# brockpat/JKMP22-Machine-Learning-and-the-Implementable-Efficient-Frontier-Replication

Measured on AMD Instinct MI355X. Metric: PFML hp×window solves/sec (whole node); full grid-search wall-clock, S&P500, higher is better.
Workload: dtype fp64; 1 GPU; global_batch=42824, seq_len=710, parallelism=dp1, dist_backend=none, device=AMD Radeon Graphics, outputs_finite=True, includes_s4_inputs=False, ridge_solve_dtype=fp64 (lambda = 0 / rank-deficient systems: bf16 cannot carry them, SURVEY 7.4), hip_graph=True

## Files before the change

### jkmp22-machine-learning-and-the-implementable-efficient-frontier-replication_amd/csrc/segsum.hip

```cpp
#include "common.h"

namespace {

__device__ __forceinline__ double* seg_slot(double* out, double* scratch, int g, int s, int nseg,
                                            int skip, int64_t PP) {
  return s < skip ? scratch + ((int64_t)g * skip + s) * PP
                  : out + ((int64_t)g * (nseg - skip) + (s - skip)) * PP;
}

__global__ __launch_bounds__(256) void wsum_upper_kernel(const double* __restrict__ X, int P,
                                                         int T, const int* __restrict__ seg_start,
                                                         const int* __restrict__ seg_stop,
                                                         int nseg, int skip,
                                                         double* __restrict__ out,
                                                         double* __restrict__ scratch) {
  const int i = blockIdx.x, s = blockIdx.y, g = blockIdx.z;
  const int a = seg_start[s], b = seg_stop[s];
  const int64_t PP = (int64_t)P * P;
  const double* src = X + (int64_t)g * T * PP + (int64_t)i * P;
  double* dst = seg_slot(out, scratch, g, s, nseg, skip, PP) + (int64_t)i * P;
  for (int j = i + threadIdx.x; j < P; j += 256) {
    double acc[4] = {0.0, 0.0, 0.0, 0.0};
    int tm = a;
    for (; tm + 4 <= b; tm += 4) {
#pragma unroll
      for (int u = 0; u < 4; ++u) acc[u] += src[(int64_t)(tm + u) * PP + j];
    }
    for (; tm < b; ++tm) acc[0] += src[(int64_t)tm * PP + j];
    dst[j] = (acc[0] + acc[1]) + (acc[2] + acc[3]);
  }
}

constexpr int WV_COLS = 64, WV_SEG = 128, WV_T = 1024, WV_RG = WV_T / WV_COLS;
template <int COLS, int RG>
__device__ __forceinline__ void wvec_segsums(const double* src, int64_t E, const int* seg_start,
                                             const int* seg_stop, int nseg, int ry, int lc,
                                             double (*part)[COLS]) {
  for (int s = ry; s < nseg; s += RG) {
    const int a = seg_start[s], b = seg_stop[s];
    double acc[8] = {0.0, 0.0, 0.0, 0.0, 0.0, 0.0, 0.0, 0.0};
    for (int tm = a; tm < b; tm += 8) {
      double x[8];
#pragma unroll
      for (int u = 0; u < 8; ++u) x[u] = (tm + u < b) ? src[(int64_t)(tm + u) * E] : 0.0;
#pragma unroll
      for (int u = 0; u < 8; ++u) acc[u] += x[u];
    }
    part[s][lc] = ((acc[0] + acc[1]) + (acc[2] + acc[3])) + ((acc[4] + acc[5]) + (acc[6] + acc[7]));
  }
}

}

namespace {

__device__ __forceinline__ bool tile_upper(int I, int J, int i, int j, int r, int c, int P) {
  return i < P && j < P && (I != J || c >= r);
}

__global__ __launch_bounds__(256) void wsum_chunk_totals_kernel(
    int P, int nseg, int skip, const double* __restrict__ out, const double* __restrict__ scratch,
    int nlc, const int* __restrict__ cs, const int* __restrict__ ce, const int* __restrict__ slot,
    double* __restrict__ tot, int64_t tstride) {
  const int g = blockIdx.y, lc = blockIdx.z;
  int tile = blockIdx.x;
  const int nt = (P + 31) / 32;
  int I = 0;
  while (tile >= nt - I) { tile -= nt - I; ++I; }
  const int J = I + tile;
  const int64_t PP = (int64_t)P * P;
  const int t = threadIdx.x, c = t & 31, r0 = t >> 5;
  double acc[4] = {0.0, 0.0, 0.0, 0.0};
  const int s0 = cs[lc], s1 = ce[lc];
  double nx[4];
  auto fetch = [&](int s) {
    const double* o = seg_slot(const_cast<double*>(out), const_cast<double*>(scratch), g, s,
                               nseg, skip, PP);
#pragma unroll
    for (int q = 0; q < 4; ++q) {
      const int i = min(I * 32 + r0 + 8 * q, P - 1), j = min(J * 32 + c, P - 1);
      nx[q] = o[(int64_t)i * P + j];
    }
  };
  if (s0 < s1) fetch(s0);
  for (int s = s0; s < s1; ++s) {
    double cur[4];
#pragma unroll
    for (int q = 0; q < 4; ++q) cur[q] = nx[q];
    if (s + 1 < s1) fetch(s + 1);
#pragma unroll
    for (int q = 0; q < 4; ++q) {
      const int r = r0 + 8 * q, i = I * 32 + r, j = J * 32 + c;
      if (tile_upper(I, J, i, j, r, c, P)) acc[q] += cur[q];
    }
  }
  double* d = tot + (int64_t)slot[lc] * tstride + (int64_t)g * PP;
#pragma unroll
  for (int q = 0; q < 4; ++q) {
    const int r = r0 + 8 * q, i = I * 32 + r, j = J * 32 + c;
    if (tile_upper(I, J, i, j, r, c, P)) d[(int64_t)i * P + j] = acc[q];
  }
}

__global__ __launch_bounds__(256) void wsum_chunk_prefix_kernel(
    int P, int nseg, int skip, double* __restrict__ out, double* __restrict__ scratch, int C,
    const int* __restrict__ sb, const int* __restrict__ sy, const int* __restrict__ ys,
    const int* __restrict__ ye, const double* __restrict__ tot, int64_t tstride, int clast) {
  __shared__ double Ts[32][33];
  const int g = blockIdx.y, ch = blockIdx.z;
  const int s0 = ys[ch], s1 = ye[ch];
  if (s0 >= s1) return;
  int tile = blockIdx.x;
  const int nt = (P + 31) / 32;
  int I = 0;
  while (tile >= nt - I) { tile -= nt - I; ++I; }
  const int J = I + tile;
  const int64_t PP = (int64_t)P * P;
  const int t = threadIdx.x, c = t & 31, r0 = t >> 5;
  const double* tg = tot + (int64_t)g * PP;
  double nx[4];
  auto fetch = [&](int s) {
    const double* o = seg_slot(out, scratch, g, s, nseg, skip, PP);
#pragma unroll
    for (int q = 0; q < 4; ++q) {
      const int i = min(I * 32 + r0 + 8 * q, P - 1), j = min(J * 32 + c, P - 1);
      nx[q] = o[(int64_t)i * P + j];
    }
  };
  fetch(s0);
  double acc[4] = {0.0, 0.0, 0.0, 0.0};
  const int nk = C + ch;
  for (int k0 = 0; k0 < nk; k0 += 8) {
    double v[8][4];
#pragma unroll
    for (int u = 0; u < 8; ++u) {
      const int k = min(k0 + u, nk - 1);
      const double* o = tg + (int64_t)(k < C ? sb[k] : sy[k - C]) * tstride;
#pragma unroll
      for (int q = 0; q < 4; ++q) {
        const int i = min(I * 32 + r0 + 8 * q, P - 1), j = min(J * 32 + c, P - 1);
        v[u][q] = o[(int64_t)i * P + j];
      }
    }
#pragma unroll
    for (int u = 0; u < 8; ++u) {
      if (k0 + u < nk) {
#pragma unroll
        for (int q = 0; q < 4; ++q) {
          const int r = r0 + 8 * q, i = I * 32 + r, j = J * 32 + c;
          if (tile_upper(I, J, i, j, r, c, P)) acc[q] += v[u][q];
        }
      }
    }
  }
  for (int s = s0; s < s1; ++s) {
    double cur[4];
#pragma unroll
    for (int q = 0; q < 4; ++q) cur[q] = nx[q];
    if (s + 1 < s1) fetch(s + 1);
#pragma unroll
    for (int q = 0; q < 4; ++q) {
      const int r = r0 + 8 * q, i = I * 32 + r, j = J * 32 + c;
      const double v = tile_upper(I, J, i, j, r, c, P) ? cur[q] : 0.0;
      acc[q] += v;
      Ts[r][c] = acc[q];
    }
    __syncthreads();
    if (s >= skip) {
      double* w = seg_slot(out, scratch, g, s, nseg, skip, PP);
#pragma unroll
      for (int q = 0; q < 4; ++q) {
        const int r = r0 + 8 * q;
        const int i = I * 32 + r, j = J * 32 + c;
        if (i < P && j < P) w[(int64_t)i * P + j] = (I != J || c >= r) ? Ts[r][c] : Ts[c][r];
        const int i2 = J * 32 + r, j2 = I * 32 + c;
        if (I != J && i2 < P && j2 < P) w[(int64_t)i2 * P + j2] = Ts[c][r];
      }
    }
    __syncthreads();
  }
}

__global__ __launch_bounds__(WV_T) void wvec_chunk_kernel(
    const double* __restrict__ X, int64_t E, int T, const int* __restrict__ seg_start,
    const int* __restrict__ seg_stop, int nseg, int skip, int mode, int nlc,
    const int* __restrict__ cs, const int* __restrict__ ce, const int* __restrict__ slot, int C,
    const int* __restrict__ sb, const int* __restrict__ sy, const int* __restrict__ ys,
    const int* __restrict__ ye, int clast, double* __restrict__ tot, int64_t tstride,
    double* __restrict__ out) {
  __shared__ double part[WV_SEG][WV_COLS];
  const int lc = threadIdx.x % WV_COLS, ry = threadIdx.x / WV_COLS;
  const int g = blockIdx.y, col = blockIdx.x * WV_COLS + lc;
  const bool cv = col < E;
  const double* src = X + (int64_t)g * T * E + (cv ? col : 0);
  wvec_segsums<WV_COLS, WV_RG>(src, E, seg_start, seg_stop, nseg, ry, lc, part);
  __syncthreads();
  if (ry != 0 || !cv) return;
  double* tg = tot + (int64_t)g * E + col;
  if (mode == 0) {
    for (int k = 0; k < nlc; ++k) {
      double acc = 0.0;
      for (int s = cs[k]; s < ce[k]; ++s) acc += part[s][lc];
      tg[(int64_t)slot[k] * tstride] = acc;
    }
    return;
  }
  double pc = 0.0;
  for (int k = 0; k < C; ++k) pc += tg[(int64_t)sb[k] * tstride];
  double* o = out + (int64_t)g * (nseg - skip) * E + col;
  for (int ch = 0; ch <= clast; ++ch) {
    double acc = pc;
    for (int s = ys[ch]; s < ye[ch]; ++s) {
      acc += part[s][lc];
      if (s >= skip) o[(int64_t)(s - skip) * E] = acc;
    }
    if (ch < clast) pc += tg[(int64_t)sy[ch] * tstride];
  }
}

}

extern "C" hipError_t pfml_wsum_chunk_totals(const double* X, int P, int T, int G,
                                             const int* seg_start, const int* seg_stop, int nseg,
                                             int skip, double* out, double* scratch, int nlc,
                                             const int* idx, double* tot, int64_t tstride,
                                             hipStream_t st) {
  if (nseg <= 0 || P <= 0 || G <= 0) return hipSuccess;
  if (skip < 0 || skip > nseg || (skip > 0 && scratch == nullptr)) return hipErrorInvalidValue;
  hipLaunchKernelGGL(wsum_upper_kernel, dim3(P, nseg, G), dim3(256), 0, st, X, P, T, seg_start,
                     seg_stop, nseg, skip, out, scratch);
  if (nlc > 0) {
    const int nt = (P + 31) / 32;
    hipLaunchKernelGGL(wsum_chunk_totals_kernel, dim3(nt * (nt + 1) / 2, G, nlc), dim3(256), 0, st, P,
                       nseg, skip, out, scratch, nlc, idx, idx + nlc, idx + 2 * nlc, tot,
                       tstride);
  }
  return hipGetLastError();
}

extern "C" hipError_t pfml_wsum_chunk_prefix(int P, int G, int nseg, int skip, double* out,
                                             double* scratch, int C, const int* cidx,
                                             const double* tot, int64_t tstride, int clast,
                                             hipStream_t st) {
  if (nseg <= 0 || P <= 0 || G <= 0 || clast < 0) return hipSuccess;
  const int nt = (P + 31) / 32;
  hipLaunchKernelGGL(wsum_chunk_prefix_kernel, dim3(nt * (nt + 1) / 2, G, clast + 1), dim3(256), 0, st, P,
                     nseg, skip, out, scratch, C, cidx, cidx + C, cidx + 2 * C, cidx + 3 * C, tot,
                     tstride, clast);
  return hipGetLastError();
}

namespace {
constexpr int OP_T = 256, OP_R = 8, OP_C = 64, OP_LD = OP_C + 2;
constexpr int OP_VC = 32, OP_VRG = OP_T / OP_VC;
static_assert(OP_T == OP_R * OP_C / 2, "one thread per column pair of the tile");
static_assert(2 * OP_R * OP_LD <= WV_SEG * OP_VC, "the tile buffers fit the vector job's LDS");

typedef double op_d2 __attribute__((ext_vector_type(2)));
struct __attribute__((aligned(8))) op_pair { double x, y; };

template <bool FULL>
__device__ __forceinline__ op_d2 op_load(const double* p, bool v0, bool v1) {
  op_d2 r = {0.0, 0.0};
  if (FULL) {
    const op_pair q = *reinterpret_cast<const op_pair*>(p);
    r.x = q.x;
    r.y = q.y;
  } else {
    if (v0) r.x = p[0];
    if (v1) r.y = p[1];
  }
  return r;
}

template <bool FULL>
__device__ __forceinline__ void op_store(double* p, bool v0, bool v1, double x, double y) {
  if (FULL) {
    op_pair q = {x, y};
    *reinterpret_cast<op_pair*>(p) = q;
  } else {
    if (v0) p[0] = x;
    if (v1) p[1] = y;
  }
}

template <bool FULL>
struct OpStream {
  const double* Xg;
  unsigned off;
  const int* seg_start;
  const int* seg_stop;
  int64_t PP;
  int nseg, ps, tm, b;
  bool v0, v1;
  op_d2 x[12];

  __device__ __forceinline__ void next() {
    tm += 12;
    while (tm >= b && ps < nseg) {
      tm = seg_start[ps];
      b = seg_stop[ps];
      ++ps;
    }
    if (tm < b) {
#pragma unroll
      for (int m = 0; m < 12; ++m)
        x[m] = op_load<FULL>(Xg + (int64_t)min(tm + m, b - 1) * PP + off, v0, v1);
    }
  }

  __device__ __forceinline__ op_d2 segsum(int a, int b1) {
    op_d2 c[4] = {{0.0, 0.0}, {0.0, 0.0}, {0.0, 0.0}, {0.0, 0.0}};
    for (int t0 = a; t0 < b1; t0 += 12) {
      if (t0 + 12 <= b1) {
#pragma unroll
        for (int m = 0; m < 12; ++m) c[m & 3] += x[m];
      } else {
        const int n = b1 - t0, n4 = n & ~3;
#pragma unroll
        for (int m = 0; m < 8; ++m) c[m & 3] += m < n4 ? x[m] : op_d2{0.0, 0.0};
#pragma unroll
        for (int m = 0; m < 11; ++m) c[0] += (m >= n4 && m < n) ? x[m] : op_d2{0.0, 0.0};
      }
      next();
    }
    return (c[0] + c[1]) + (c[2] + c[3]);
  }
};

template <bool FULL>
__device__ __forceinline__ void op_tile(const double* __restrict__ X, int P, int T, int g, int I,
                                        int J, const int* __restrict__ seg_start,
                                        const int* __restrict__ seg_stop, int nseg, int skip,
                                        const int* __restrict__ cs, const int* __restrict__ ce,
                                        int C, const int* __restrict__ sb,
                                        const int* __restrict__ ys, const int* __restrict__ ye,
                                        int clast, double* __restrict__ SD, double* Ts) {
  const int64_t PP = (int64_t)P * P;
  const int nwin = nseg - skip;
  const int t = threadIdx.x;
  const int r = t / (OP_C / 2), cp = (t % (OP_C / 2)) * 2;
  const int i = I * OP_R + r, j = J * OP_C + cp;
  const bool v0 = FULL || (i < P && j < P && j >= i);
  const bool v1 = FULL || (i < P && j + 1 < P && j + 1 >= i);
  const int tc = t / (OP_R / 2), tr = (t % (OP_R / 2)) * 2;
  const int i2 = J * OP_C + tc, j2 = I * OP_R + tr;
  const bool w0 = FULL || (i2 < P && j2 < i2);
  const bool w1 = FULL || (i2 < P && j2 + 1 < i2);
  OpStream<FULL> ms;
  ms.Xg = X + (int64_t)g * T * PP;
  ms.off = FULL || (i < P && j < P) ? (unsigned)i * P + j : 0u;
  ms.seg_start = seg_start;
  ms.seg_stop = seg_stop;
  ms.PP = PP;
  ms.nseg = nseg;
  ms.ps = 0;
  ms.tm = -12;
  ms.b = 0;
  ms.v0 = v0;
  ms.v1 = v1;
#pragma unroll
  for (int m = 0; m < 12; ++m) ms.x[m] = op_d2{0.0, 0.0};
  ms.next();
  op_d2 pc = {0.0, 0.0};
  for (int k = 0; k < C; ++k) {
    const int q = sb[k];
    op_d2 tot = {0.0, 0.0};
    for (int s = cs[q]; s < ce[q]; ++s) tot += ms.segsum(seg_start[s], seg_stop[s]);
    pc += tot;
  }
  int nst = 0;
  for (int ch = 0; ch <= clast; ++ch) {
    op_d2 acc = pc, tot = {0.0, 0.0};
    for (int s = ys[ch]; s < ye[ch]; ++s) {
      const op_d2 v = ms.segsum(seg_start[s], seg_stop[s]);
      tot += v;
      acc += v;
      if (s < skip) continue;
      double* w = SD + ((int64_t)g * nwin + (s - skip)) * PP;
      op_store<FULL>(w + (int64_t)i * P + j, v0, v1, acc.x, acc.y);
      double* tb = Ts + (nst & 1) * (OP_R * OP_LD);
      ++nst;
      tb[r * OP_LD + cp] = acc.x;
      tb[r * OP_LD + cp + 1] = acc.y;
      __syncthreads();
      op_store<FULL>(w + (int64_t)i2 * P + j2, w0, w1, tb[tr * OP_LD + tc],
                     tb[(tr + 1) * OP_LD + tc]);
    }
    if (ch < clast) pc += tot;
  }
}

__global__ __launch_bounds__(OP_T) void wsum_onepass_kernel(
    const double* __restrict__ X, const double* __restrict__ R, int P, int T,
    const int* __restrict__ seg_start, const int* __restrict__ seg_stop, int nseg, int skip,
    const int* __restrict__ cs, const int* __restrict__ ce, int C, const int* __restrict__ sb,
    const int* __restrict__ ys, const int* __restrict__ ye, int clast, int nvb,
    double* __restrict__ SD, double* __restrict__ Sr) {
  __shared__ double smem[WV_SEG * OP_VC];
  const int g = blockIdx.y, nwin = nseg - skip;
  if ((int)blockIdx.x >= nvb) {
    int tile = blockIdx.x - nvb;
    const int ntc = (P + OP_C - 1) / OP_C;
    int I = 0;
    while (tile >= ntc - I * OP_R / OP_C) { tile -= ntc - I * OP_R / OP_C; ++I; }
    const int J = I * OP_R / OP_C + tile;
    const bool full = I * OP_R + OP_R - 1 <= J * OP_C && J * OP_C + OP_C <= P;
    if (full)
      op_tile<true>(X, P, T, g, I, J, seg_start, seg_stop, nseg, skip, cs, ce, C, sb, ys, ye,
                    clast, SD, smem);
    else
      op_tile<false>(X, P, T, g, I, J, seg_start, seg_stop, nseg, skip, cs, ce, C, sb, ys, ye,
                     clast, SD, smem);
    return;
  }
  double (*part)[OP_VC] = reinterpret_cast<double (*)[OP_VC]>(smem);
  const int lc = threadIdx.x % OP_VC, ry = threadIdx.x / OP_VC;
  const int col = blockIdx.x * OP_VC + lc;
  const bool cv = col < P;
  const double* src = R + (int64_t)g * T * P + (cv ? col : 0);
  wvec_segsums<OP_VC, OP_VRG>(src, P, seg_start, seg_stop, nseg, ry, lc, part);
  __syncthreads();
  if (ry != 0 || !cv) return;
  double pc = 0.0;
  for (int k = 0; k < C; ++k) {
    const int q = sb[k];
    double tot = 0.0;
    for (int s = cs[q]; s < ce[q]; ++s) tot += part[s][lc];
    pc += tot;
  }
  double* o = Sr + (int64_t)g * nwin * P + col;
  for (int ch = 0; ch <= clast; ++ch) {
    double acc = pc, tot = 0.0;
    for (int s = ys[ch]; s < ye[ch]; ++s) {
      tot += part[s][lc];
      acc += part[s][lc];
      if (s >= skip) o[(int64_t)(s - skip) * P] = acc;
    }
    if (ch < clast) pc += tot;
  }
}

}

extern "C" hipError_t pfml_wsum_onepass(const double* X, const double* R, int P, int T, int G,
                                        const int* seg_start, const int* seg_stop, int nseg,
                                        int skip, int nlc, const int* idx, int C, const int* cidx,
                                        int clast, double* SD, double* Sr, hipStream_t st) {
  if (nseg <= 0 || P <= 0 || G <= 0 || clast < 0 || nseg - skip <= 0) return hipSuccess;
  if (nseg > WV_SEG || skip < 0 || T <= 0 || nlc != 2 * C || clast >= C || P > 65535)
    return hipErrorInvalidValue;
  const int ntr = (P + OP_R - 1) / OP_R, ntc = (P + OP_C - 1) / OP_C;
  int ntile = 0;
  for (int I = 0; I < ntr; ++I) ntile += ntc - I * OP_R / OP_C;
  const int nvb = (P + OP_VC - 1) / OP_VC;
  hipLaunchKernelGGL(wsum_onepass_kernel, dim3(nvb + ntile, G), dim3(OP_T), 0, st, X, R, P, T,
                     seg_start, seg_stop, nseg, skip, idx, idx + nlc, C, cidx, cidx + 2 * C,
                     cidx + 3 * C, clast, nvb, SD, Sr);
  return hipGetLastError();
}

extern "C" hipError_t pfml_wvec_chunk(const double* X, int64_t E, int T, int G,
                                      const int* seg_start, const int* seg_stop, int nseg,
                                      int skip, int mode, int nlc, const int* idx, int C,
                                      const int* cidx, int clast, double* tot, int64_t tstride,
                                      double* out, hipStream_t st) {
  if (nseg <= 0 || E <= 0 || G <= 0) return hipSuccess;
  if (nseg > WV_SEG || skip < 0) return hipErrorInvalidValue;
  if (mode == 1 && (clast < 0 || nseg - skip <= 0)) return hipSuccess;
  if (mode == 0 && nlc <= 0) return hipSuccess;
  hipLaunchKernelGGL(wvec_chunk_kernel, dim3((unsigned)((E + WV_COLS - 1) / WV_COLS), G),
                     dim3(WV_T), 0, st, X, E, T, seg_start, seg_stop, nseg, skip, mode, nlc, idx,
                     idx + nlc, idx + 2 * nlc, C, cidx, cidx + C, cidx + 2 * C, cidx + 3 * C,
                     clast, tot, tstride, out);
  return hipGetLastError();
}
```

### jkmp22-machine-learning-and-the-implementable-efficient-frontier-replication_amd/ops/wsum.py

```python
from __future__ import annotations

import ctypes as C
from dataclasses import dataclass

import numpy as np
import torch

from . import _native as nat

MAX_SEGMENTS = 128

nat.register_hip("pfml_wsum_chunk_totals", [C.c_void_p, C.c_int, C.c_int, C.c_int, C.c_void_p,
                                            C.c_void_p, C.c_int, C.c_int, C.c_void_p, C.c_void_p,
                                            C.c_int, C.c_void_p, C.c_void_p, C.c_int64,
                                            C.c_void_p])
nat.register_hip("pfml_wsum_chunk_prefix", [C.c_int, C.c_int, C.c_int, C.c_int, C.c_void_p,
                                            C.c_void_p, C.c_int, C.c_void_p, C.c_void_p,
                                            C.c_int64, C.c_int, C.c_void_p])
nat.register_hip("pfml_wvec_chunk", [C.c_void_p, C.c_int64, C.c_int, C.c_int, C.c_void_p,
                                     C.c_void_p, C.c_int, C.c_int, C.c_int, C.c_int, C.c_void_p,
                                     C.c_int, C.c_void_p, C.c_int, C.c_void_p, C.c_int64,
                                     C.c_void_p, C.c_void_p])
nat.register_hip("pfml_wsum_onepass", [C.c_void_p, C.c_void_p, C.c_int, C.c_int, C.c_int,
                                       C.c_void_p, C.c_void_p, C.c_int, C.c_int, C.c_int,
                                       C.c_void_p, C.c_int, C.c_void_p, C.c_int, C.c_void_p,
                                       C.c_void_p, C.c_void_p])


@dataclass(frozen=True, eq=False)
class WindowPlan:
    T: int
    nseg: int
    skip: int
    nYl: int
    nlc: int
    C: int
    clast: int
    counts: tuple
    st: np.ndarray
    sp: np.ndarray
    cs: np.ndarray
    ce: np.ndarray
    slot: np.ndarray
    sb: np.ndarray
    sy: np.ndarray
    ys: np.ndarray
    ye: np.ndarray
    onepass: bool
    d_st: torch.Tensor | None = None
    d_sp: torch.Tensor | None = None
    d_cs_ce_slot: torch.Tensor | None = None
    d_sb_sy_ys_ye: torch.Tensor | None = None

    @property
    def nslot(self) -> int:
        return int(sum(self.counts))


def window_plan(*, T: int, skip: int, C: int, clast: int, counts, st, sp, cs, ce, slot, sb, sy,
                ys, ye, dev=None, who: str = "window plan") -> WindowPlan:
    st, sp, cs, ce, slot, sb, sy, ys, ye = (np.asarray(a, np.int32) for a in
                                            (st, sp, cs, ce, slot, sb, sy, ys, ye))
    nseg, nlc, nslot = len(st), len(cs), int(sum(counts))
    if nseg and (st.min() < 0 or sp.max() > T or (sp < st).any() or nseg > MAX_SEGMENTS):
        raise ValueError(f"{who}: window segments out of range (T={T}, nseg={nseg})")
    for a, b in ((cs, ce), (ys, ye)):
        if len(a) and (a.min() < 0 or b.max() > nseg or (b < a).any()):
            raise ValueError(f"{who}: chunk segment ranges out of range")
    for arr in (sb, sy):
        if len(arr) and (arr.min() < 0 or arr.max() >= nslot):
            raise ValueError(f"{who}: chunk total slots out of range")
    if len(slot) and (slot.min() < 0 or slot.max() >= nlc):
        raise ValueError(f"{who}: local chunk slots out of range")
    nYl = nseg - skip
    onepass = nlc == nslot and nlc == 2 * C and np.array_equal(slot, np.arange(nlc))
    if onepass:
        walk = ([s for k in range(C) for s in range(cs[sb[k]], ce[sb[k]])]
                + [s for c in range(clast + 1) for s in range(ys[c], ye[c])])
        own = sy[:clast + 1]
        onepass = (walk == list(range(nseg)) and np.array_equal(cs[own], ys[:clast + 1])
                   and np.array_equal(ce[own], ye[:clast + 1]))
    d = [None] * 4
    if nseg and dev is not None and dev.type == "cuda":
        d = nat.upload([st, sp, np.concatenate([cs, ce, slot]),
                        np.concatenate([sb, sy, ys, ye])], dev)
    return WindowPlan(T=int(T), nseg=nseg, skip=int(skip), nYl=nYl, nlc=nlc, C=int(C),
                      clast=int(clast), counts=tuple(int(c) for c in counts), st=st, sp=sp,
                      cs=cs, ce=ce, slot=slot, sb=sb, sy=sy, ys=ys, ye=ye, onepass=bool(onepass),
                      d_st=d[0], d_sp=d[1], d_cs_ce_slot=d[2], d_sb_sy_ys_ye=d[3])


def _fold_months(X: torch.Tensor, a: int, b: int) -> torch.Tensor:
    acc = torch.zeros_like(X[:, 0])
    for t in range(a, b):
        acc = acc + X[:, t]
    return acc


def chunk_totals(X: torch.Tensor, R: torch.Tensor, wp: WindowPlan):
    G, T, P, _ = X.shape
    nlc, nseg, skip = wp.nlc, wp.nseg, wp.skip
    GPP = G * P * P
    tot = torch.empty((nlc, GPP + G * P), dtype=X.dtype, device=X.device)
    totD = tot[:, :GPP].view(nlc, G, P, P)
    totR = tot[:, GPP:].view(nlc, G, P)
    out = torch.empty((G, wp.nYl, P, P), dtype=X.dtype, device=X.device)
    if nat.is_device(X):
        if X.dtype != torch.float64 or not X.is_contiguous():
            raise ValueError("chunk_totals: contiguous fp64 required")
        scratch = (torch.empty((G, skip, P, P), dtype=X.dtype, device=X.device) if skip
                   else None)
        lib = nat.hip_lib()
        s = nat.stream_of(X)
        nat.check(lib.pfml_wsum_chunk_totals(
            X.data_ptr(), P, T, G, nat.ptr(wp.d_st), nat.ptr(wp.d_sp), nseg, skip,
            out.data_ptr(), nat.ptr(scratch), nlc, nat.ptr(wp.d_cs_ce_slot), totD.data_ptr(),
            totD.stride(0), s), "pfml_wsum_chunk_totals")
        nat.check(lib.pfml_wvec_chunk(
            R.data_ptr(), P, T, G, nat.ptr(wp.d_st), nat.ptr(wp.d_sp), nseg, skip, 0, nlc,
            nat.ptr(wp.d_cs_ce_slot), wp.C, nat.ptr(wp.d_sb_sy_ys_ye), wp.clast,
            totR.data_ptr(), totR.stride(0), None, s), "pfml_wvec_chunk")
        return totD, totR, {"out": out, "scratch": scratch, "tot": tot}
    segD = [_fold_months(X, a, b) for a, b in zip(wp.st, wp.sp)]
    segR = [_fold_months(R, a, b) for a, b in zip(wp.st, wp.sp)]
    for lc in range(nlc):
        accD, accR = torch.zeros_like(X[:, 0]), torch.zeros_like(R[:, 0])
        for s in range(int(wp.cs[lc]), int(wp.ce[lc])):
            accD = accD + segD[s]
            accR = accR + segR[s]
        totD[lc], totR[lc] = accD, accR
    return totD, totR, {"out": out, "segD": segD, "segR": segR, "tot": tot}


def chunk_windows(X: torch.Tensor, R: torch.Tensor, wp: WindowPlan, totD: torch.Tensor,
                  totR: torch.Tensor, bufs: dict) -> tuple[torch.Tensor, torch.Tensor]:
    G, T, P, _ = X.shape
    nseg, skip, clast, C = wp.nseg, wp.skip, wp.clast, wp.C
    out = bufs["out"]
    if totD.shape[0] != wp.nslot or totR.shape[0] != wp.nslot:
        raise ValueError(f"chunk_windows: {totD.shape[0]} chunk totals, the canonical layout "
                         f"has {wp.nslot} slots (all-gather missing?)")
    Sr = torch.empty((G, wp.nYl, P), dtype=X.dtype, device=X.device)
    if nat.is_device(X):
        lib = nat.hip_lib()
        s = nat.stream_of(X)
        if totD.stride()[1:] != (P * P, P, 1) or totR.stride()[1:] != (P, 1):
            raise ValueError("chunk_windows: chunk totals must be row-strided [slot][g] blocks")
        nat.check(lib.pfml_wsum_chunk_prefix(
            P, G, nseg, skip, out.data_ptr(), nat.ptr(bufs["scratch"]), C,
            nat.ptr(wp.d_sb_sy_ys_ye), totD.data_ptr(), totD.stride(0), clast, s),
            "pfml_wsum_chunk_prefix")
        nat.check(lib.pfml_wvec_chunk(
            R.data_ptr(), P, T, G, nat.ptr(wp.d_st), nat.ptr(wp.d_sp), nseg, skip, 1, 0,
            nat.ptr(wp.d_cs_ce_slot), C, nat.ptr(wp.d_sb_sy_ys_ye), clast, totR.data_ptr(),
            totR.stride(0), Sr.data_ptr(), s), "pfml_wvec_chunk")
        return out, Sr
    segD, segR = bufs["segD"], bufs["segR"]
    pD, pR = torch.zeros_like(X[:, 0]), torch.zeros_like(R[:, 0])
    for k in range(C):
        pD = pD + totD[int(wp.sb[k])]
        pR = pR + totR[int(wp.sb[k])]
    for c in range(clast + 1):
        aD, aR = pD, pR
        for s in range(int(wp.ys[c]), int(wp.ye[c])):
            aD = aD + segD[s]
            aR = aR + segR[s]
            if s >= skip:
                out[:, s - skip] = aD
                Sr[:, s - skip] = aR
        if c < clast:
            pD = pD + totD[int(wp.sy[c])]
            pR = pR + totR[int(wp.sy[c])]
    return out, Sr


def window_sums_onepass(X: torch.Tensor, R: torch.Tensor, wp: WindowPlan):
    G, T, P, _ = X.shape
    if not nat.is_device(X) or not nat.is_device(R):
        raise ValueError("window_sums_onepass: device tensors required")
    if X.dtype != torch.float64 or not X.is_contiguous():
        raise ValueError("window_sums_onepass: contiguous fp64 required")
    if R.dtype != torch.float64 or not R.is_contiguous() or R.shape != (G, T, P):
        raise ValueError("window_sums_onepass: R must be a contiguous fp64 [G, T, P] tensor")
    if not wp.onepass or T != wp.T:
        raise ValueError("window_sums_onepass: this rank does not own every chunk of the "
                         "canonical layout (world size one required)")
    SD = torch.empty((G, wp.nYl, P, P), dtype=X.dtype, device=X.device)
    Sr = torch.empty((G, wp.nYl, P), dtype=X.dtype, device=X.device)
    if wp.nYl == 0 or wp.nseg == 0:
        return SD, Sr
    nat.check(nat.hip_lib().pfml_wsum_onepass(
        X.data_ptr(), R.data_ptr(), P, T, G, nat.ptr(wp.d_st), nat.ptr(wp.d_sp), wp.nseg,
        wp.skip, wp.nlc, nat.ptr(wp.d_cs_ce_slot), wp.C, nat.ptr(wp.d_sb_sy_ys_ye), wp.clast,
        SD.data_ptr(), Sr.data_ptr(), nat.stream_of(X)), "pfml_wsum_onepass")
    return SD, Sr
```

Baseline: 10.10 million solves/s.

## Schedule one-pass window sums from a balanced host-built work-unit table

The fixed 8x64 tile grid of the one-pass window-sum kernel is replaced by a host-computed table of work units. The table cuts each 8-row band of the upper triangle into variable-width column strips so per-block work is roughly equal, sized to a target number of units per compute unit. Paired 16-byte loads and stores now apply to any even-width off-diagonal strip rather than only full tiles. A timed kernel variant and census helpers are added for inspection. The cost is an extra device table lookup per block, and the table must be built eagerly before graph capture.

```diff
diff --git a/jkmp22-machine-learning-and-the-implementable-efficient-frontier-replication_amd/csrc/segsum.hip b/jkmp22-machine-learning-and-the-implementable-efficient-frontier-replication_amd/csrc/segsum.hip
--- a/jkmp22-machine-learning-and-the-implementable-efficient-frontier-replication_amd/csrc/segsum.hip
+++ b/jkmp22-machine-learning-and-the-implementable-efficient-frontier-replication_amd/csrc/segsum.hip
@@ -253,19 +253,22 @@
 namespace {
 constexpr int OP_T = 256, OP_R = 8, OP_C = 64, OP_LD = OP_C + 2;
 constexpr int OP_VC = 32, OP_VRG = OP_T / OP_VC;
+constexpr int OP_VECTOR = -1;
 static_assert(OP_T == OP_R * OP_C / 2, "one thread per column pair of the tile");
 static_assert(2 * OP_R * OP_LD <= WV_SEG * OP_VC, "the tile buffers fit the vector job's LDS");
 
 typedef double op_d2 __attribute__((ext_vector_type(2)));
 struct __attribute__((aligned(8))) op_pair { double x, y; };
 
-template <bool FULL>
+template <bool PAIR>
 __device__ __forceinline__ op_d2 op_load(const double* p, bool v0, bool v1) {
   op_d2 r = {0.0, 0.0};
-  if (FULL) {
-    const op_pair q = *reinterpret_cast<const op_pair*>(p);
-    r.x = q.x;
-    r.y = q.y;
+  if (PAIR) {
+    if (v0) {
+      const op_pair q = *reinterpret_cast<const op_pair*>(p);
+      r.x = q.x;
+      r.y = q.y;
+    }
   } else {
     if (v0) r.x = p[0];
     if (v1) r.y = p[1];
@@ -273,18 +276,20 @@
   return r;
 }
 
-template <bool FULL>
+template <bool PAIR>
 __device__ __forceinline__ void op_store(double* p, bool v0, bool v1, double x, double y) {
-  if (FULL) {
-    op_pair q = {x, y};
-    *reinterpret_cast<op_pair*>(p) = q;
+  if (PAIR) {
+    if (v0) {
+      op_pair q = {x, y};
+      *reinterpret_cast<op_pair*>(p) = q;
+    }
   } else {
     if (v0) p[0] = x;
     if (v1) p[1] = y;
   }
 }
 
-template <bool FULL>
+template <bool PAIR>
 struct OpStream {
   const double* Xg;
   unsigned off;
@@ -305,7 +310,7 @@
     if (tm < b) {
 #pragma unroll
       for (int m = 0; m < 12; ++m)
-        x[m] = op_load<FULL>(Xg + (int64_t)min(tm + m, b - 1) * PP + off, v0, v1);
+        x[m] = op_load<PAIR>(Xg + (int64_t)min(tm + m, b - 1) * PP + off, v0, v1);
     }
   }
 
@@ -328,9 +333,9 @@
   }
 };
 
-template <bool FULL>
-__device__ __forceinline__ void op_tile(const double* __restrict__ X, int P, int T, int g, int I,
-                                        int J, const int* __restrict__ seg_start,
+template <bool PAIR>
+__device__ __forceinline__ void op_unit(const double* __restrict__ X, int P, int T, int g, int i0,
+                                        int c0, int w, const int* __restrict__ seg_start,
                                         const int* __restrict__ seg_stop, int nseg, int skip,
                                         const int* __restrict__ cs, const int* __restrict__ ce,
                                         int C, const int* __restrict__ sb,
@@ -340,16 +345,16 @@
   const int nwin = nseg - skip;
   const int t = threadIdx.x;
   const int r = t / (OP_C / 2), cp = (t % (OP_C / 2)) * 2;
-  const int i = I * OP_R + r, j = J * OP_C + cp;
-  const bool v0 = FULL || (i < P && j < P && j >= i);
-  const bool v1 = FULL || (i < P && j + 1 < P && j + 1 >= i);
+  const int i = i0 + r, j = c0 + cp;
+  const bool v0 = PAIR ? cp < w : (i < P && cp < w && j >= i);
+  const bool v1 = PAIR ? v0 : (i < P && cp + 1 < w && j + 1 >= i);
   const int tc = t / (OP_R / 2), tr = (t % (OP_R / 2)) * 2;
-  const int i2 = J * OP_C + tc, j2 = I * OP_R + tr;
-  const bool w0 = FULL || (i2 < P && j2 < i2);
-  const bool w1 = FULL || (i2 < P && j2 + 1 < i2);
-  OpStream<FULL> ms;
+  const int i2 = c0 + tc, j2 = i0 + tr;
+  const bool w0 = PAIR ? tc < w : (tc < w && j2 < i2);
+  const bool w1 = PAIR ? w0 : (tc < w && j2 + 1 < i2);
+  OpStream<PAIR> ms;
   ms.Xg = X + (int64_t)g * T * PP;
-  ms.off = FULL || (i < P && j < P) ? (unsigned)i * P + j : 0u;
+  ms.off = v0 || v1 ? (unsigned)i * P + j : 0u;
   ms.seg_start = seg_start;
   ms.seg_stop = seg_stop;
   ms.PP = PP;
@@ -377,46 +382,45 @@
       tot += v;
       acc += v;
       if (s < skip) continue;
-      double* w = SD + ((int64_t)g * nwin + (s - skip)) * PP;
-      op_store<FULL>(w + (int64_t)i * P + j, v0, v1, acc.x, acc.y);
+      double* win = SD + ((int64_t)g * nwin + (s - skip)) * PP;
+      op_store<PAIR>(win + (int64_t)i * P + j, v0, v1, acc.x, acc.y);
       double* tb = Ts + (nst & 1) * (OP_R * OP_LD);
       ++nst;
       tb[r * OP_LD + cp] = acc.x;
       tb[r * OP_LD + cp + 1] = acc.y;
       __syncthreads();
-      op_store<FULL>(w + (int64_t)i2 * P + j2, w0, w1, tb[tr * OP_LD + tc],
+      op_store<PAIR>(win + (int64_t)i2 * P + j2, w0, w1, tb[tr * OP_LD + tc],
                      tb[(tr + 1) * OP_LD + tc]);
     }
     if (ch < clast) pc += tot;
   }
 }
 
-__global__ __launch_bounds__(OP_T) void wsum_onepass_kernel(
-    const double* __restrict__ X, const double* __restrict__ R, int P, int T,
+__device__ __forceinline__ void op_work(
+    const double* __restrict__ X, const double* __restrict__ R, int P, int T, int G,
     const int* __restrict__ seg_start, const int* __restrict__ seg_stop, int nseg, int skip,
     const int* __restrict__ cs, const int* __restrict__ ce, int C, const int* __restrict__ sb,
-    const int* __restrict__ ys, const int* __restrict__ ye, int clast, int nvb,
-    double* __restrict__ SD, double* __restrict__ Sr) {
-  __shared__ double smem[WV_SEG * OP_VC];
-  const int g = blockIdx.y, nwin = nseg - skip;
-  if ((int)blockIdx.x >= nvb) {
-    int tile = blockIdx.x - nvb;
-    const int ntc = (P + OP_C - 1) / OP_C;
-    int I = 0;
-    while (tile >= ntc - I * OP_R / OP_C) { tile -= ntc - I * OP_R / OP_C; ++I; }
-    const int J = I * OP_R / OP_C + tile;
-    const bool full = I * OP_R + OP_R - 1 <= J * OP_C && J * OP_C + OP_C <= P;
-    if (full)
-      op_tile<true>(X, P, T, g, I, J, seg_start, seg_stop, nseg, skip, cs, ce, C, sb, ys, ye,
-                    clast, SD, smem);
+    const int* __restrict__ ys, const int* __restrict__ ye, int clast,
+    const int4* __restrict__ units, double* __restrict__ SD, double* __restrict__ Sr,
+    double* smem) {
+  const int4 u = units[blockIdx.x];
+  const int g = u.x, nwin = nseg - skip;
+  if (g < 0 || g >= G) return;
+  if (u.y != OP_VECTOR) {
+    const int i0 = u.y, c0 = u.z, w = u.w;
+    if (i0 < 0 || c0 < i0 || w < 1 || w > OP_C || c0 + w > P) return;
+    if (c0 >= i0 + OP_R && (w & 1) == 0)
+      op_unit<true>(X, P, T, g, i0, c0, w, seg_start, seg_stop, nseg, skip, cs, ce, C, sb, ys,
+                    ye, clast, SD, smem);
     else
-      op_tile<false>(X, P, T, g, I, J, seg_start, seg_stop, nseg, skip, cs, ce, C, sb, ys, ye,
-                     clast, SD, smem);
+      op_unit<false>(X, P, T, g, i0, c0, w, seg_start, seg_stop, nseg, skip, cs, ce, C, sb, ys,
+                     ye, clast, SD, smem);
     return;
   }
+  if (u.z < 0 || u.z * OP_VC >= P) return;
   double (*part)[OP_VC] = reinterpret_cast<double (*)[OP_VC]>(smem);
   const int lc = threadIdx.x % OP_VC, ry = threadIdx.x / OP_VC;
-  const int col = blockIdx.x * OP_VC + lc;
+  const int col = u.z * OP_VC + lc;
   const bool cv = col < P;
   const double* src = R + (int64_t)g * T * P + (cv ? col : 0);
   wvec_segsums<OP_VC, OP_VRG>(src, P, seg_start, seg_stop, nseg, ry, lc, part);
@@ -441,23 +445,70 @@
   }
 }
 
+
+template <bool TIMED>
+__global__ __launch_bounds__(OP_T) void wsum_onepass_kernel(
+    const double* __restrict__ X, const double* __restrict__ R, int P, int T, int G,
+    const int* __restrict__ seg_start, const int* __restrict__ seg_stop, int nseg, int skip,
+    const int* __restrict__ cs, const int* __restrict__ ce, int C, const int* __restrict__ sb,
+    const int* __restrict__ ys, const int* __restrict__ ye, int clast,
+    const int4* __restrict__ units, double* __restrict__ SD, double* __restrict__ Sr,
+    long long* __restrict__ dbg) {
+  __shared__ double smem[WV_SEG * OP_VC];
+  long long t0 = 0;
+  if (TIMED && threadIdx.x == 0) t0 = (long long)wall_clock64();
+  op_work(X, R, P, T, G, seg_start, seg_stop, nseg, skip, cs, ce, C, sb, ys, ye, clast, units, SD,
+          Sr, smem);
+  if (TIMED) {
+    __syncthreads();
+    if (threadIdx.x == 0) {
+      long long* d = dbg + 4 * (int64_t)blockIdx.x;
+      d[0] = t0;
+      d[1] = (long long)wall_clock64();
+      d[2] = __builtin_amdgcn_s_getreg(4 | (31 << 11));
+      d[3] = __builtin_amdgcn_s_getreg(20 | (31 << 11));
+    }
+  }
+}
+
+}
+
+namespace {
+template <bool TIMED>
+hipError_t wsum_onepass_launch(const double* X, const double* R, int P, int T, int G,
+                               const int* seg_start, const int* seg_stop, int nseg, int skip,
+                               int nlc, const int* idx, int C, const int* cidx, int clast,
+                               double* SD, double* Sr, hipStream_t st, const int* units,
+                               int nunits, long long* dbg) {
+  if (nseg <= 0 || P <= 0 || G <= 0 || clast < 0 || nseg - skip <= 0) return hipSuccess;
+  if (nseg > WV_SEG || skip < 0 || T <= 0 || nlc != 2 * C || clast >= C || P > 65535 ||
+      units == nullptr || nunits <= 0)
+    return hipErrorInvalidValue;
+  hipLaunchKernelGGL(wsum_onepass_kernel<TIMED>, dim3(nunits), dim3(OP_T), 0, st, X, R, P, T, G,
+                     seg_start, seg_stop, nseg, skip, idx, idx + nlc, C, cidx, cidx + 2 * C,
+                     cidx + 3 * C, clast, reinterpret_cast<const int4*>(units), SD, Sr, dbg);
+  return hipGetLastError();
+}
 }
 
 extern "C" hipError_t pfml_wsum_onepass(const double* X, const double* R, int P, int T, int G,
                                         const int* seg_start, const int* seg_stop, int nseg,
                                         int skip, int nlc, const int* idx, int C, const int* cidx,
-                                        int clast, double* SD, double* Sr, hipStream_t st) {
-  if (nseg <= 0 || P <= 0 || G <= 0 || clast < 0 || nseg - skip <= 0) return hipSuccess;
-  if (nseg > WV_SEG || skip < 0 || T <= 0 || nlc != 2 * C || clast >= C || P > 65535)
-    return hipErrorInvalidValue;
-  const int ntr = (P + OP_R - 1) / OP_R, ntc = (P + OP_C - 1) / OP_C;
-  int ntile = 0;
-  for (int I = 0; I < ntr; ++I) ntile += ntc - I * OP_R / OP_C;
-  const int nvb = (P + OP_VC - 1) / OP_VC;
-  hipLaunchKernelGGL(wsum_onepass_kernel, dim3(nvb + ntile, G), dim3(OP_T), 0, st, X, R, P, T,
-                     seg_start, seg_stop, nseg, skip, idx, idx + nlc, C, cidx, cidx + 2 * C,
-                     cidx + 3 * C, clast, nvb, SD, Sr);
-  return hipGetLastError();
+                                        int clast, double* SD, double* Sr, hipStream_t st,
+                                        const int* units, int nunits) {
+  return wsum_onepass_launch<false>(X, R, P, T, G, seg_start, seg_stop, nseg, skip, nlc, idx, C,
+                                    cidx, clast, SD, Sr, st, units, nunits, nullptr);
+}
+
+extern "C" hipError_t pfml_wsum_onepass_timed(const double* X, const double* R, int P, int T,
+                                              int G, const int* seg_start, const int* seg_stop,
+                                              int nseg, int skip, int nlc, const int* idx, int C,
+                                              const int* cidx, int clast, double* SD, double* Sr,
+                                              hipStream_t st, const int* units, int nunits,
+                                              long long* dbg) {
+  if (dbg == nullptr) return hipErrorInvalidValue;
+  return wsum_onepass_launch<true>(X, R, P, T, G, seg_start, seg_stop, nseg, skip, nlc, idx, C,
+                                   cidx, clast, SD, Sr, st, units, nunits, dbg);
 }
 
 extern "C" hipError_t pfml_wvec_chunk(const double* X, int64_t E, int T, int G,
diff --git a/jkmp22-machine-learning-and-the-implementable-efficient-frontier-replication_amd/ops/wsum.py b/jkmp22-machine-learning-and-the-implementable-efficient-frontier-replication_amd/ops/wsum.py
--- a/jkmp22-machine-learning-and-the-implementable-efficient-frontier-replication_amd/ops/wsum.py
+++ b/jkmp22-machine-learning-and-the-implementable-efficient-frontier-replication_amd/ops/wsum.py
@@ -1,7 +1,7 @@
 from __future__ import annotations
 
 import ctypes as C
-from dataclasses import dataclass
+from dataclasses import dataclass, field
 
 import numpy as np
 import torch
@@ -21,10 +21,169 @@
                                      C.c_void_p, C.c_int, C.c_int, C.c_int, C.c_int, C.c_void_p,
                                      C.c_int, C.c_void_p, C.c_int, C.c_void_p, C.c_int64,
                                      C.c_void_p, C.c_void_p])
-nat.register_hip("pfml_wsum_onepass", [C.c_void_p, C.c_void_p, C.c_int, C.c_int, C.c_int,
-                                       C.c_void_p, C.c_void_p, C.c_int, C.c_int, C.c_int,
-                                       C.c_void_p, C.c_int, C.c_void_p, C.c_int, C.c_void_p,
-                                       C.c_void_p, C.c_void_p])
+_ONEPASS_ARGS = [C.c_void_p, C.c_void_p, C.c_int, C.c_int, C.c_int, C.c_void_p, C.c_void_p,
+                 C.c_int, C.c_int, C.c_int, C.c_void_p, C.c_int, C.c_void_p, C.c_int, C.c_void_p,
+                 C.c_void_p, C.c_void_p, C.c_void_p, C.c_int]
+nat.register_hip("pfml_wsum_onepass", _ONEPASS_ARGS)
+
+
+def onepass_timed_entry():
+    lib = nat.hip_lib()
+    if not hasattr(lib, "pfml_wsum_onepass_timed"):
+        return None
+    fn = lib.pfml_wsum_onepass_timed
+    fn.argtypes, fn.restype = _ONEPASS_ARGS + [C.c_void_p], C.c_int
+    return fn
+
+
+TIMED_WORDS = 4
+
+UNIT_ROWS, UNIT_COLS, UNIT_VCOLS = 8, 64, 32
+UNIT_MIN_COLS = 16
+UNIT_PER_CU = 3
+UNIT_VECTOR = -1
+UNIT_LEVEL_BOUND = 1.20
+
+
+def _band_cut(i0: int, nr: int, P: int, n: int):
+    L = P - i0
+    if n == 1:
+        return [(i0, L)] if L <= UNIT_COLS else None
+    tri = nr * (nr - 1) // 2
+    wd = int(round(((nr * L - tri) / n + tri) / nr))
+    wd += (L - wd) & 1
+    wd = max(1 + (L + 1) % 2, min(wd, UNIT_COLS - (L - UNIT_COLS) % 2, L - 2 * (n - 1)))
+    pairs = (L - wd) // 2
+    q, r = divmod(pairs, n - 1)
+    if wd < 1 or (L - wd) & 1 or q < 1 or 2 * (q + (r > 0)) > UNIT_COLS:
+        return None
+    out, c0 = [(i0, wd)], i0 + wd
+    for k in range(n - 1):
+        w = 2 * (q + (k < r))
+        out.append((c0, w))
+        c0 += w
+    return out
+
+
+def _bands(P: int, room: int):
+    import heapq
+    band, heap = {}, []
+    for i0 in range(0, P, UNIT_ROWS):
+        nr, L = min(UNIT_ROWS, P - i0), P - i0
+        n = -(-L // UNIT_COLS)
+        while _band_cut(i0, nr, P, n) is None:
+            n += 1
+        band[i0] = n
+        heapq.heappush(heap, (-(nr * L - nr * (nr - 1) // 2) / n, i0))
+    left = room - sum(band.values())
+    while left > 0 and heap:
+        _, i0 = heapq.heappop(heap)
+        nr, L, n = min(UNIT_ROWS, P - i0), P - i0, band[i0] + 1
+        if L // n < UNIT_MIN_COLS or _band_cut(i0, nr, P, n) is None:
+            continue
+        band[i0] = n
+        left -= 1
+        heapq.heappush(heap, (-(nr * L - nr * (nr - 1) // 2) / n, i0))
+    return [(i0, _band_cut(i0, min(UNIT_ROWS, P - i0), P, n)) for i0, n in sorted(band.items())]
+
+
+def unit_table(P: int, G: int, ncu: int = 256, per_cu: int = UNIT_PER_CU) -> np.ndarray:
+    if P < 1 or G < 1:
+        raise ValueError("unit_table: P and G must be positive")
+    nvb = -(-P // UNIT_VCOLS)
+    bands = _bands(P, (per_cu * ncu - G * nvb) // G)
+    rows = [(g, i0, c0, w) for g in range(G) for i0, cut in bands for c0, w in cut]
+    vec = [(g, UNIT_VECTOR, b, min(UNIT_VCOLS, P - b * UNIT_VCOLS)) for g in range(G)
+           for b in range(nvb)]
+    rows += vec
+    return np.asarray(rows, dtype=np.int32).reshape(-1, 4)
+
+
+def check_units(units: np.ndarray, P: int, G: int) -> None:
+    u = np.asarray(units)
+    if u.ndim != 2 or u.shape[1] != 4 or u.dtype != np.int32 or len(u) == 0:
+        raise ValueError("unit table: [n, 4] int32 required")
+    g, i0, c0, w = u.T
+    vec = i0 == UNIT_VECTOR
+    ok = (g >= 0) & (g < G) & (w >= 1)
+    ok &= np.where(vec, (c0 >= 0) & (c0 * UNIT_VCOLS < P) & (w <= UNIT_VCOLS),
+                   (i0 >= 0) & (i0 % UNIT_ROWS == 0) & (c0 >= i0) & (w <= UNIT_COLS)
+                   & (c0 + w <= P))
+    if not ok.all():
+        raise ValueError(f"unit table: unit {int(np.flatnonzero(~ok)[0])} out of range "
+                         f"(P={P}, G={G})")
+
+
+def unit_lanes(unit, P: int):
+    _, i0, c0, w = (int(v) for v in unit)
+    pair = c0 >= i0 + UNIT_ROWS and w % 2 == 0
+    read, mirror = [], []
+    for t in range(UNIT_ROWS * UNIT_COLS // 2):
+        r, cp = t // (UNIT_COLS // 2), (t % (UNIT_COLS // 2)) * 2
+        i, j = i0 + r, c0 + cp
+        tc, tr = t // (UNIT_ROWS // 2), (t % (UNIT_ROWS // 2)) * 2
+        i2, j2 = c0 + tc, i0 + tr
+        if pair:
+            v = [cp < w, cp < w]
+            m = [tc < w, tc < w]
+        else:
+            v = [i < P and cp + e < w and j + e >= i for e in (0, 1)]
+            m = [tc < w and j2 + e < i2 for e in (0, 1)]
+        read += [(i, j + e) for e in (0, 1) if v[e]]
+        mirror += [(i2, j2 + e) for e in (0, 1) if m[e]]
+    return read, mirror
+
+
+def unit_costs(units: np.ndarray, P: int) -> np.ndarray:
+    out = np.empty(len(units), dtype=np.int64)
+    for k, (_, i0, c0, w) in enumerate(np.asarray(units).tolist()):
+        if i0 == UNIT_VECTOR:
+            out[k] = w
+        else:
+            out[k] = sum(max(0, c0 + w - max(c0, i)) for i in range(i0, min(i0 + UNIT_ROWS, P)))
+    return out
+
+
+def unit_kinds(units: np.ndarray) -> list:
+    out = []
+    for _, i0, c0, w in np.asarray(units).tolist():
+        if i0 == UNIT_VECTOR:
+            out.append("vector")
+        elif c0 == i0:
+            out.append("diagonal")
+        elif c0 >= i0 + UNIT_ROWS and w % 2 == 0:
+            out.append("full" if w == UNIT_COLS else "pair")
+        else:
+            out.append("masked")
+    return out
+
+
+def tile_census(P: int, G: int = 1):
+    kinds, costs, TR, TC = [], [], 8, 64
+    ntc = -(-P // TC)
+    for b in range(-(-P // UNIT_VCOLS)):
+        kinds.append("vector")
+        costs.append(min(UNIT_VCOLS, P - b * UNIT_VCOLS))
+    for i0 in range(0, P, TR):
+        for J in range(i0 // TC, ntc):
+            c0, c1 = J * TC, min(P, (J + 1) * TC)
+            n = sum(max(0, c1 - max(c0, i)) for i in range(i0, min(i0 + TR, P)))
+            whole = i0 + TR - 1 <= c0 and c1 - c0 == TC
+            kinds.append("full" if whole else "diagonal" if c0 <= i0 + TR - 1 else "strip")
+            costs.append(n)
+    return kinds * G, np.asarray(costs * G, dtype=np.int64)
+
+
+def census(kinds, costs) -> dict:
+    costs = np.asarray(costs, dtype=np.int64)
+    tot = max(1, int(costs.sum()))
+    per = {}
+    for k in dict.fromkeys(kinds):
+        c = costs[[x == k for x in kinds]]
+        per[k] = {"count": int(len(c)), "share": float(c.sum()) / tot, "min": int(c.min()),
+                  "max": int(c.max())}
+    return {"n": int(len(costs)), "kinds": per, "max": int(costs.max()),
+            "mean": float(costs.mean()), "max_over_mean": float(costs.max() / costs.mean())}
 
 
 @dataclass(frozen=True, eq=False)
@@ -51,10 +210,29 @@
     d_sp: torch.Tensor | None = None
     d_cs_ce_slot: torch.Tensor | None = None
     d_sb_sy_ys_ye: torch.Tensor | None = None
+    units: dict = field(default_factory=dict)
 
     @property
     def nslot(self) -> int:
         return int(sum(self.counts))
+
+    def onepass_units(self, P: int, G: int, dev) -> tuple:
+        key = (int(P), int(G), str(dev))
+        hit = self.units.get(key)
+        if hit is None:
+            if torch.cuda.is_current_stream_capturing():
+                raise RuntimeError("window plan: the one-pass unit table of this shape must "
+                                   "be built by an eager run before the step is captured")
+            units = unit_table(P, G, ncu=torch.cuda.get_device_properties(dev)
+                               .multi_processor_count)
+            check_units(units, P, G)
+            hit = (units, nat.upload([units], dev)[0])
+            self.units[key] = hit
+        return hit
+
+    def levelness(self, P: int, G: int, ncu: int = 256) -> dict:
+        units = unit_table(P, G, ncu=ncu)
+        return census(unit_kinds(units), unit_costs(units, P))
 
 
 def window_plan(*, T: int, skip: int, C: int, clast: int, counts, st, sp, cs, ce, slot, sb, sy,
@@ -189,8 +367,10 @@
     Sr = torch.empty((G, wp.nYl, P), dtype=X.dtype, device=X.device)
     if wp.nYl == 0 or wp.nseg == 0:
         return SD, Sr
+    units, d_units = wp.onepass_units(P, G, X.device)
     nat.check(nat.hip_lib().pfml_wsum_onepass(
         X.data_ptr(), R.data_ptr(), P, T, G, nat.ptr(wp.d_st), nat.ptr(wp.d_sp), wp.nseg,
         wp.skip, wp.nlc, nat.ptr(wp.d_cs_ce_slot), wp.C, nat.ptr(wp.d_sb_sy_ys_ye), wp.clast,
-        SD.data_ptr(), Sr.data_ptr(), nat.stream_of(X)), "pfml_wsum_onepass")
+        SD.data_ptr(), Sr.data_ptr(), nat.stream_of(X), nat.ptr(d_units), len(units)),
+        "pfml_wsum_onepass")
     return SD, Sr
```

Measured after the change: 10.14 million solves/s, median of 3. About the same (+0.3%).
